# hzdr/PARIS

Hardware: AMD Instinct MI355X
Metric: GVoxel-updates/s (voxels x projections / s), FDK hot path weight+filter+backproject (higher is better)
Workload: dtype f32

## Files before the change

include/paris_hip.h:

```cpp
#ifndef PARIS_HIP_H_
#define PARIS_HIP_H_

#include <stddef.h>
#include <stdint.h>

#ifdef __cplusplus
extern "C" {
#endif

#define PARIS_HIP_SUCCESS 0
#define PARIS_HIP_ERROR_INVALID_ARGUMENT 10001
#define PARIS_HIP_ERROR_NO_DEVICE 10002
#define PARIS_HIP_ERROR_UNSUPPORTED 10003

#define PARIS_HIP_CTX_DEFAULT 0u
#define PARIS_HIP_CTX_SYNCHRONOUS 1u
#define PARIS_HIP_CTX_LEGACY_STREAM 2u
#define PARIS_HIP_CTX_WARM 4u

typedef struct paris_detector_geometry {
    uint32_t n_row;
    uint32_t n_col;
    float l_px_row;
    float l_px_col;
// ... 215 lines not shown
int paris_hip_stage_backproject(paris_hip_ctx* ctx, const float* d_p, size_t p_pitch, uint32_t p_dim_x,
                                uint32_t p_dim_y, uint32_t p_idx, float p_phi, float* d_v, uint32_t v_dim_x,
                                uint32_t v_dim_y, uint32_t v_dim_z, uint32_t v_offset,
                                const paris_detector_geometry* det_geo, const paris_volume_geometry* vol_geo,
                                int enable_angles, int enable_roi, const paris_region_of_interest* roi);

int paris_hip_forward_project(paris_hip_ctx* ctx, const float* d_v, uint32_t v_dim_x, uint32_t v_dim_y, uint32_t v_dim_z,
                              uint32_t v_offset, const paris_detector_geometry* det_geo, const paris_volume_geometry* vol_geo,
                              float* d_p, size_t p_pitch, size_t p_stride_bytes, uint32_t n_views, uint32_t p_dim_x,
                              uint32_t p_dim_y, const float* sin_phi, const float* cos_phi, float delta_s, float delta_t,
                              int accumulate);
int paris_hip_stage_forward_project(paris_hip_ctx* ctx, const float* d_v, uint32_t v_dim_x, uint32_t v_dim_y, uint32_t v_dim_z,
                                    uint32_t v_offset, const paris_detector_geometry* det_geo, const paris_volume_geometry* vol_geo,
                                    float* d_p, size_t p_pitch, uint32_t p_dim_x, uint32_t p_dim_y, uint32_t p_idx, float p_phi,
                                    int enable_angles, int accumulate);

const char* paris_hip_strerror(int status);
const char* paris_hip_version(void);
int paris_hip_has_experiments(void);
int paris_hip_last_backproject_ms(paris_hip_ctx* ctx, float* ms);
int paris_hip_backproject_timing_arm(paris_hip_ctx* ctx, uint32_t capacity);
int paris_hip_backproject_timing_collect(paris_hip_ctx* ctx, float* ms, uint32_t max_n, uint32_t* n_out);
int paris_hip_set_backproject_variant(paris_hip_ctx* ctx, int variant);
int paris_hip_set_backproject_tuning(paris_hip_ctx* ctx, int vx, int unroll, int tz, int lds_bytes);
int paris_hip_set_backproject_slice_shape(paris_hip_ctx* ctx, int waves, int row_groups);
int paris_hip_set_backproject_order(paris_hip_ctx* ctx, int order, int nontemporal);
int paris_hip_set_backproject_fast_division(paris_hip_ctx* ctx, int enable);
int paris_hip_set_backproject_vector_staging(paris_hip_ctx* ctx, int enable);
int paris_hip_fast_division_is_exact(paris_hip_ctx* ctx, float divisor, int* exact);
int paris_hip_lean_division_is_exact(paris_hip_ctx* ctx, float d_sd, float d_so, int* exact);
int paris_hip_lean_weighting_is_exact(paris_hip_ctx* ctx, float d_sd, float q_lo, float q_hi, int* exact);
int paris_hip_set_lean_validation(paris_hip_ctx* ctx, int enable);

#ifdef __cplusplus
}
#endif
#endif
```

paris_amd/_lib.py:

```python
import ctypes as C
import os

_HERE = os.path.dirname(os.path.abspath(__file__))
EXPERIMENTS_LIB_PATH = os.path.join(_HERE, "lib", "libparis_hip_experiments.so")
LIB_PATH = os.environ.get("PARIS_HIP_LIBRARY") or os.path.join(_HERE, "lib", "libparis_hip.so")

SUCCESS = 0
ERROR_INVALID_ARGUMENT = 10001
ERROR_NO_DEVICE = 10002
ERROR_UNSUPPORTED = 10003
CTX_DEFAULT = 0
CTX_SYNCHRONOUS = 1
CTX_LEGACY_STREAM = 2
CTX_WARM = 4
PIXEL_U8 = 1
PIXEL_U16 = 2
PIXEL_U32 = 3
PIXEL_F32 = 4


class DetectorGeometry(C.Structure):
    _fields_ = [("n_row", C.c_uint32), ("n_col", C.c_uint32),
                ("l_px_row", C.c_float), ("l_px_col", C.c_float),
                ("delta_s", C.c_float), ("delta_t", C.c_float),
# ... 127 lines not shown
                                          _P(RegionOfInterest), _P(_u32), _P(_u32)]),
    "paris_hip_stage_angle": (C.c_int, [_P(DetectorGeometry), _u32, C.c_int, _f, _P(_f), _P(_f)]),
    "paris_hip_short_scan_check": (C.c_int, [_P(DetectorGeometry), _P(ShortScan), _P(_f)]),
    "paris_hip_short_scan_weight_rows": (C.c_int, [_vp, _vp, _sz, _sz, _u32, _u32, _u32, _u32, _u32, _P(DetectorGeometry), _P(ShortScan),
                                                   _P(_f)]),
    "paris_hip_stage_short_scan_weight": (C.c_int, [_vp, _vp, _sz, _u32, _u32, _P(DetectorGeometry), _P(ShortScan), _u32, C.c_int,
                                                    _f]),
    "paris_hip_offset_detector_check": (C.c_int, [_P(DetectorGeometry), _P(_f)]),
    "paris_hip_offset_detector_weight_rows": (C.c_int, [_vp, _vp, _sz, _sz, _u32, _u32, _u32, _u32, _u32, _P(DetectorGeometry)]),
    "paris_hip_stage_offset_detector_weight": (C.c_int, [_vp, _vp, _sz, _u32, _u32, _P(DetectorGeometry)]),
    "paris_hip_stage_backproject": (C.c_int, [_vp, _vp, _sz, _u32, _u32, _u32, _f, _vp, _u32, _u32, _u32, _u32,
                                              _P(DetectorGeometry), _P(VolumeGeometry), C.c_int, C.c_int,
                                              _P(RegionOfInterest)]),
    "paris_hip_forward_project": (C.c_int, [_vp, _vp, _u32, _u32, _u32, _u32, _P(DetectorGeometry), _P(VolumeGeometry), _vp, _sz, _sz,
                                            _u32, _u32, _u32, _P(_f), _P(_f), _f, _f, C.c_int]),
    "paris_hip_stage_forward_project": (C.c_int, [_vp, _vp, _u32, _u32, _u32, _u32, _P(DetectorGeometry), _P(VolumeGeometry), _vp, _sz,
                                                  _u32, _u32, _u32, _f, C.c_int, C.c_int]),
    "paris_hip_strerror": (C.c_char_p, [C.c_int]),
    "paris_hip_version": (C.c_char_p, []),
    "paris_hip_last_backproject_ms": (C.c_int, [_vp, _P(_f)]),
    "paris_hip_backproject_timing_arm": (C.c_int, [_vp, _u32]),
    "paris_hip_backproject_timing_collect": (C.c_int, [_vp, _P(_f), _u32, _P(_u32)]),
    "paris_hip_set_backproject_variant": (C.c_int, [_vp, C.c_int]),
    "paris_hip_set_backproject_tuning": (C.c_int, [_vp, C.c_int, C.c_int, C.c_int, C.c_int]),
    "paris_hip_set_backproject_order": (C.c_int, [_vp, C.c_int, C.c_int]),
    "paris_hip_set_backproject_slice_shape": (C.c_int, [_vp, C.c_int, C.c_int]),
    "paris_hip_set_backproject_fast_division": (C.c_int, [_vp, C.c_int]),
    "paris_hip_set_backproject_vector_staging": (C.c_int, [_vp, C.c_int]),
    "paris_hip_fast_division_is_exact": (C.c_int, [_vp, _f, _P(C.c_int)]),
}

_lib = None


def load():
    global _lib
    if _lib is None:
        if not os.path.exists(LIB_PATH):
            raise ImportError(
                "paris_amd: %s not found -- build it with `python -c 'import __graft_entry__ as g; g.build()'` "
                "or `make -C paris_amd/csrc`; there is no CPU fallback" % LIB_PATH)
        if os.environ.get("PARIS_AMD_NO_TORCH") != "1":
            try:
                import torch
            except ImportError:
                pass
        lib = C.CDLL(LIB_PATH)
# ... 24 lines not shown
```

paris_amd/backend.py:

```python
import ctypes as C

import numpy as np

from . import _lib
from ._lib import (DefectStats, DetectorGeometry, ParisHipError, RegionOfInterest, ShortScan, SubvolumeGeometry, SubvolumeInfo,
                   VolumeGeometry, check)

__all__ = ["DetectorGeometry", "VolumeGeometry", "SubvolumeGeometry", "RegionOfInterest", "SubvolumeInfo",
           "ParisHipError", "ShortScan", "Projection", "Volume", "FilterBuffer", "Backend", "get_devices", "set_device",
           "calculate_volume_geometry", "apply_roi", "filter_size", "load", "make_volume", "weight", "filter",
           "backproject", "forward_project", "short_scan_check", "offset_detector_check", "DefectPlan", "defect_plan"]


class Projection:

    def __init__(self, buf, dim_x, dim_y, idx=0, phi=0.0, pitch=None, on_device=False, owner=None):
        self.buf = buf
        self.dim_x = dim_x
        self.dim_y = dim_y
        self.idx = idx
        self.phi = phi
        self.pitch = pitch if pitch is not None else dim_x * 4
        self.on_device = on_device
        self._owner = owner
# ... 398 lines not shown
        check(self._L.paris_hip_forward_project(self._ctx, v.ptr, v.dim_x, v.dim_y, v.dim_z, v_offset, C.byref(det_geo), C.byref(vol_geo),
                                                p.ptr, p.pitch, frame_stride, len(sins), p.dim_x, p.dim_y, sins.ctypes.data_as(fp),
                                                coss.ctypes.data_as(fp), delta_s, delta_t, int(bool(accumulate))),
              "paris_hip_forward_project")

    def last_backproject_ms(self):
        ms = C.c_float()
        check(self._L.paris_hip_last_backproject_ms(self._ctx, C.byref(ms)), "paris_hip_last_backproject_ms")
        return ms.value

    def backproject_timing_arm(self, capacity):
        check(self._L.paris_hip_backproject_timing_arm(self._ctx, capacity), "paris_hip_backproject_timing_arm")

    def backproject_timing_collect(self, max_n=65536):
        ms = (C.c_float * max_n)()
        n = C.c_uint32()
        check(self._L.paris_hip_backproject_timing_collect(self._ctx, ms, max_n, C.byref(n)),
              "paris_hip_backproject_timing_collect")
        return list(ms[:n.value])

    def set_backproject_variant(self, variant):
        check(self._L.paris_hip_set_backproject_variant(self._ctx, variant), "paris_hip_set_backproject_variant")

    def set_backproject_order(self, order=-1, nontemporal=-1):
        check(self._L.paris_hip_set_backproject_order(self._ctx, order, nontemporal), "paris_hip_set_backproject_order")

    def fast_division_is_exact(self, divisor):
        ok = C.c_int()
        check(self._L.paris_hip_fast_division_is_exact(self._ctx, divisor, C.byref(ok)), "paris_hip_fast_division_is_exact")
        return bool(ok.value)

    def set_backproject_vector_staging(self, enable=True):
        check(self._L.paris_hip_set_backproject_vector_staging(self._ctx, int(bool(enable))),
              "paris_hip_set_backproject_vector_staging")

    def set_backproject_fast_division(self, enable=True):
        check(self._L.paris_hip_set_backproject_fast_division(self._ctx, int(bool(enable))),
              "paris_hip_set_backproject_fast_division")

    def set_backproject_slice_shape(self, waves=0, row_groups=0):
        check(self._L.paris_hip_set_backproject_slice_shape(self._ctx, waves, row_groups),
              "paris_hip_set_backproject_slice_shape")

    def set_filter_window(self, window):
        check(self._L.paris_hip_set_filter_window(self._ctx, window), "paris_hip_set_filter_window")

# ... 168 lines not shown
```

paris_amd/csrc/backproject.hip:

```cpp
#include "bp_device.h"

#include <mutex>
#include <utility>

namespace
{
    __global__ void __launch_bounds__(256) fastdiv_validate_kernel(float c, float r, unsigned long long* mismatches)
    {
        const uint32_t t = blockIdx.x * 256u + threadIdx.x;
        unsigned int bad = 0;
        for(uint32_t i = 0; i < 256u; ++i)
        {
            const uint32_t bits = (i << 24) | t;
            const float x = __uint_as_float(bits);
            const float want = x / c - (1.f / 2.f);
            const float got = div_by_constant(x, c, r) - (1.f / 2.f);
            const bool same = __float_as_uint(want) == __float_as_uint(got);
            const bool both_nan = (want != want) && (got != got);
            const bool want_far = !(fabsf(want) <= 16777216.f);
            const bool got_far = !(fabsf(got) <= 16777216.f);
            if(!(same || both_nan || (want_far && got_far)))
                ++bad;
        }
        if(bad)
            atomicAdd(mismatches, static_cast<unsigned long long>(bad));
    }

#ifndef PARIS_TILE_MIN_WAVES
#define PARIS_TILE_MIN_WAVES 1
#endif
    template <int VX, int UNROLL, bool NT, bool FD, bool PRE = false>
    __global__ void __launch_bounds__(256, PARIS_TILE_MIN_WAVES) bp_tile_kernel(const BpParams g)
    {
        extern __shared__ __attribute__((aligned(16))) float lds[];

        constexpr uint32_t XL = 64u / VX;
        constexpr uint32_t RW = VX;
        constexpr uint32_t TY = 4u * RW;

        const uint32_t tid = threadIdx.x;
        const uint32_t lane = tid & 63u;
        const uint32_t wave = tid >> 6;

        uint32_t bx, by, bz;
        if(!tile_of_block(g, blockIdx.x, bx, by, bz))
            return;
        const uint32_t k0 = bx * 64u;
        const uint32_t l0 = by * TY;
        const uint32_t m0 = bz * g.tz;
        const uint32_t k1 = min(k0 + 63u, g.v_dim_x - 1u);
        const uint32_t l1 = min(l0 + TY - 1u, g.v_dim_y - 1u);
        const uint32_t m1 = min(m0 + g.tz - 1u, g.v_dim_z - 1u);

        const uint32_t xq = lane % XL;
        const uint32_t yy = lane / XL;
        const uint32_t k = k0 + xq * VX;
        const uint32_t l = l0 + wave * RW + yy;
        const bool active = k < g.v_dim_x && l < g.v_dim_y;

        float4 pre_f = make_float4(0.f, 0.f, 0.f, 0.f), pre_h = pre_f, pre_u = pre_f;
        if(PRE && VX == 4)
        {
            const size_t plane = static_cast<size_t>(g.v_dim_x) * g.v_dim_y;
            const size_t at = static_cast<size_t>(min(l, l1)) * g.v_dim_x + min(k, g.v_dim_x - 4u);
            pre_f = *reinterpret_cast<const float4*>(g.colstate + at);
            pre_h = *reinterpret_cast<const float4*>(g.colstate + plane + at);
            pre_u = *reinterpret_cast<const float4*>(g.colstate + 2u * plane + at);
        }
// ... 64 lines not shown
                    for(int i = 0; i < UNROLL; ++i)
                        acc[i] = load_voxels<VX, NT>(vp + (mm + i) * slice);
#pragma unroll
                    for(int i = 0; i < UNROLL; ++i)
                        update(acc[i], mm + i);
#pragma unroll
                    for(int i = 0; i < UNROLL; ++i)
                        store_voxels<VX, NT>(vp + (mm + i) * slice, acc[i], g.store_sc1 != 0u);
                }
                for(; mm < mcount; ++mm)
                {
                    vec_t acc = load_voxels<VX, NT>(vp + mm * slice);
                    update(acc, mm);
                    store_voxels<VX, NT>(vp + mm * slice, acc, g.store_sc1 != 0u);
                }
            }
        };
        if(all_fast)
            walk(std::true_type{});
        else
            walk(std::false_type{});
    }

#ifdef PARIS_HIP_EXPERIMENTS
#include "experiments/bp_kernels.inc"
#endif
    __global__ void __launch_bounds__(256) bp_gather_kernel(const BpParams g)
    {
        const uint32_t k = blockIdx.x * 256u + threadIdx.x;
        const uint32_t l = blockIdx.y;
        const uint32_t m = blockIdx.z;
        if(k >= g.v_dim_x)
            return;
        const ColConst c = column_constants<false>(g, g.k_off + k, g.l_off + l);
        const float z_m = g.z_base + static_cast<float>(g.m_off + m) * g.l_vx_z;
        const float x = c.h;
        const float y = v_coordinate<false>(g, z_m, c.factor);
        const float x1 = floorf(x), x2 = x1 + 1.f, y1 = floorf(y), y2 = y1 + 1.f;
        float interp = 0.f;
        if(x1 >= 0.f && x2 < g.p_dim_x_f && y1 >= 0.f && y2 < g.p_dim_y_f)
        {
            const size_t at = static_cast<size_t>(static_cast<uint32_t>(y1)) * g.p_pitch + static_cast<uint32_t>(x1);
            const float q11 = read_pixel(g, at), q21 = read_pixel(g, at + 1);
            const float q12 = read_pixel(g, at + g.p_pitch), q22 = read_pixel(g, at + g.p_pitch + 1);
            const float interp_y1 = (x2 - x) / (x2 - x1) * q11 + (x - x1) / (x2 - x1) * q21;
            const float interp_y2 = (x2 - x) / (x2 - x1) * q12 + (x - x1) / (x2 - x1) * q22;
            interp = (y2 - y) / (y2 - y1) * interp_y1 + (y - y1) / (y2 - y1) * interp_y2;
        }
        float* out = g.vol + (static_cast<size_t>(m) * g.v_dim_y + l) * g.v_dim_x + k;
        *out += 0.5f * interp * c.u * c.u;
    }

    inline float centered_base(uint32_t dim, float size)
    {
        const float size2 = size / 2.f;
        return -(static_cast<float>(dim) * size2) + size2;
    }

    inline float detector_min(uint32_t dim, float size, float offset)
    {
        const float size2 = size / 2.f;
        return -(static_cast<float>(dim) * size2) - offset;
    }

    constexpr uint32_t TZ_DEFAULT = 16;
    constexpr uint32_t LDS_BYTES_DEFAULT = 24u * 1024u;
    constexpr uint32_t LDS_BYTES_MAX = 64u * 1024u;

    template <int VX, int UNROLL, bool NT, bool FD>
    void launch_tile(BpParams& g, hipStream_t stream)
    {
        constexpr uint32_t TY = 4u * VX;
        g.ntx = (g.v_dim_x + 63u) / 64u;
        g.nty = (g.v_dim_y + TY - 1u) / TY;
        g.ntz = (g.v_dim_z + g.tz - 1u) / g.tz;
        settle_order(g);
        g.zchunk = chunk_tiles(g.order, g.tz, g.ntz, 64u);
        const uint32_t blocks = static_cast<uint32_t>(grid_blocks(g));
        hipLaunchKernelGGL((bp_tile_kernel<VX, UNROLL, NT, FD>), dim3(blocks), dim3(256), g.lds_floats * sizeof(float), stream, g);
    }

    template <int VX, bool NT, bool FD>
    void launch_tile_unroll(BpParams& g, int unroll, hipStream_t stream)
    {
        switch(unroll)
        {
            case 1: launch_tile<VX, 1, NT, FD>(g, stream); break;
#ifdef PARIS_HIP_EXPERIMENTS
            case 3: launch_tile<VX, 3, NT, FD>(g, stream); break;
            case 4: launch_tile<VX, 4, NT, FD>(g, stream); break;
#endif
            default: launch_tile<VX, 2, NT, FD>(g, stream); break;
        }
    }

    template <int VX>
    void launch_tile_flags(BpParams& g, int unroll, bool nt, bool fd, hipStream_t stream)
    {
        if(nt && fd)
            launch_tile_unroll<VX, true, true>(g, unroll, stream);
        else if(nt)
            launch_tile_unroll<VX, true, false>(g, unroll, stream);
        else if(fd)
            launch_tile_unroll<VX, false, true>(g, unroll, stream);
        else
            launch_tile_unroll<VX, false, false>(g, unroll, stream);
    }

#ifdef PARIS_HIP_EXPERIMENTS
#include "experiments/bp_launchers.inc"
#endif
    std::mutex fastdiv_mutex;
    std::map<std::pair<int, uint32_t>, bool> fastdiv_cache;

    void fastdiv_enqueue(hipStream_t s, unsigned long long* counter, const void* arg)
    {
        const float c = *static_cast<const float*>(arg);
        hipLaunchKernelGGL(fastdiv_validate_kernel, dim3(1u << 16), dim3(256), 0, s, c, 1.f / c, counter);
    }

    int fastdiv_is_exact(paris_hip_ctx* ctx, float c, bool* ok)
    {
        *ok = false;
        if(!(c > 0.f) || !(c < INFINITY))
            return PARIS_HIP_SUCCESS;
        uint32_t key;
        static_assert(sizeof(key) == sizeof(c), "fp32");
        std::memcpy(&key, &c, sizeof(key));
        auto it = ctx->fastdiv_exact.find(key);
// ... 161 lines not shown
    if(v_dim_x % 2u == 0 && addr % 8u == 0)
        return 2;
    return 1;
}

static int backproject_impl(paris_hip_ctx* ctx, const void* d_p, bool f16, size_t p_pitch, uint32_t p_dim_x,
                            uint32_t p_dim_y, float* d_v, uint32_t v_dim_x, uint32_t v_dim_y, uint32_t v_dim_z,
                            uint32_t v_offset, const paris_detector_geometry* det_geo,
                            const paris_volume_geometry* vol_geo, int enable_roi, const paris_region_of_interest* roi,
                            float sin_phi, float cos_phi, float delta_s, float delta_t)
{
    BpParams g;
    bool fd = false, skip = false;
    if(int rc = fill_params(ctx, d_p, f16, p_pitch, p_dim_x, p_dim_y, d_v, v_dim_x, v_dim_y, v_dim_z, v_offset, det_geo, vol_geo,
                            enable_roi, roi, sin_phi, cos_phi, delta_s, delta_t, g, fd, skip))
        return rc;
    if(skip)
        return paris_hip_finish(ctx);

    const bool timed = !ctx->bp_start.empty();
    const size_t ev = timed ? static_cast<size_t>(ctx->bp_launches % ctx->bp_start.size()) : 0u;
    if(timed)
        PARIS_HIP_TRY(hipEventRecord(ctx->bp_start[ev], ctx->stream));
    if(ctx->bp_variant == 4 && !f16)
    {
        FusedParams fp{};
        fp.g = g;
        fp.n_proj = 1;
        fp.proj_tab[0] = d_p;
        fp.sin_phi[0] = sin_phi;
        fp.cos_phi[0] = cos_phi;
        const int width = lane_width(d_v, v_dim_x);
        const int vx = ctx->bp_vx == 4 && width == 4 ? 4 : (ctx->bp_vx == 1 || width < 2 ? 1 : 2);
        paris_hip_bp_launch_fused(&fp, vx, ctx->bp_tz == 8u ? 8 : (ctx->bp_tz == 32u ? 32 : 16), volume_stream_policy(ctx, v_dim_x, v_dim_y, v_dim_z) != 0, fd, ctx->stream);
    }
    else
    if(ctx->bp_variant == 1)
    {
        const dim3 grid((v_dim_x + 255u) / 256u, v_dim_y, v_dim_z);
        if(v_dim_y > 65535u || v_dim_z > 65535u)
            return PARIS_HIP_ERROR_UNSUPPORTED;
        hipLaunchKernelGGL(bp_gather_kernel, grid, dim3(256), 0, ctx->stream, g);
    }
    else
    {
        int vx = lane_width(d_v, v_dim_x);
        if(ctx->bp_vx && ctx->bp_vx < vx)
            vx = ctx->bp_vx;
        if(ctx->bp_vx == 0 && vx == 4 && ctx->bp_variant != 3 && ctx->bp_variant != 5)
        {
            const uint64_t tiles = static_cast<uint64_t>((v_dim_x + 63u) / 64u) * ((v_dim_y + 15u) / 16u) * ((v_dim_z + g.tz - 1u) / g.tz);
            if(tiles < 2048u)
                vx = 2;
        }
        const bool deep_big = g.tz == 16u && ctx->bp_tz == 0u && static_cast<uint64_t>(v_dim_x) * v_dim_y > (1ull << 20);
        if(deep_big && ctx->bp_unroll == 0 && ctx->bp_lds_bytes == 0u && vx == 4)
            g.lds_floats = 40u * 1024u / sizeof(float);
        const int unroll = ctx->bp_unroll ? ctx->bp_unroll : ((g.tz == 8u && ctx->bp_tz == 0u) || (deep_big && ctx->bp_lds_bytes == 0u && vx == 4) ? 1 : 2);
        const bool nt = volume_stream_policy(ctx, v_dim_x, v_dim_y, v_dim_z) != 0;
#ifdef PARIS_HIP_EXPERIMENTS
        const bool want_slice = ctx->bp_variant == 3;
        if(want_slice && vx == 4)
        {
            const int nw = ctx->bp_slice_nw ? ctx->bp_slice_nw : 16;
            const int rpl = ctx->bp_slice_rpl ? ctx->bp_slice_rpl : 4;
            const uint32_t box_bytes = ctx->bp_lds_bytes ? ctx->bp_lds_bytes : LDS_BYTES_DEFAULT;
            if(int rc = launch_slice_shape(g, nw, rpl, box_bytes, nt, fd, ctx->stream))
                return rc;
        }
        else if(vx == 4 && ctx->bp_variant == 5 && v_dim_y <= 65535u)
        {
            const size_t need = 3u * static_cast<size_t>(v_dim_x) * v_dim_y;
            if(ctx->colstate_floats < need)
            {
                if(ctx->colstate != nullptr)
                {
                    PARIS_HIP_TRY(hipStreamSynchronize(ctx->stream));
                    PARIS_HIP_TRY(hipFree(ctx->colstate));
                    ctx->colstate = nullptr;
                }
                PARIS_HIP_TRY(hipMalloc(reinterpret_cast<void**>(&ctx->colstate), need * sizeof(float)));
                ctx->colstate_floats = need;
            }
            g.colstate = ctx->colstate;
            if(unroll == 1)
                fd ? launch_tile_pre<1, true>(g, ctx->stream) : launch_tile_pre<1, false>(g, ctx->stream);
            else
                fd ? launch_tile_pre<2, true>(g, ctx->stream) : launch_tile_pre<2, false>(g, ctx->stream);
        }
        else
#endif
        if(vx == 4)
            launch_tile_flags<4>(g, unroll, nt, fd, ctx->stream);
        else if(vx == 2)
            launch_tile_flags<2>(g, unroll, nt, fd, ctx->stream);
        else
            launch_tile_flags<1>(g, unroll, nt, fd, ctx->stream);
    }
    if(timed)
        PARIS_HIP_TRY(hipEventRecord(ctx->bp_stop[ev], ctx->stream));
    ++ctx->bp_launches;
    if(int rc = paris_hip_note_projection_use(ctx, d_p, p_pitch * p_dim_y))
        return rc;
    return paris_hip_finish(ctx);
}

static int batch_impl(paris_hip_ctx* ctx, const void* d_p, bool f16, size_t p_pitch, size_t p_stride_bytes, uint32_t n_proj, uint32_t p_dim_x,
                      uint32_t p_dim_y, float* d_v, uint32_t v_dim_x, uint32_t v_dim_y, uint32_t v_dim_z, uint32_t v_offset,
                      const paris_detector_geometry* det_geo, const paris_volume_geometry* vol_geo, int enable_roi,
                      const paris_region_of_interest* roi, const float* sin_phi, const float* cos_phi, float delta_s, float delta_t,
                      const void* const* ptrs = nullptr);

int paris_hip_launch_deferred(paris_hip_ctx* ctx)
{
    if(ctx != nullptr && ctx->pending_weight.active)
        if(int rc = paris_hip_flush_pending_weight(ctx))
            return rc;
    if(ctx == nullptr || ctx->defer_count == 0)
        return PARIS_HIP_SUCCESS;
    const uint32_t n = ctx->defer_count;
// ... 604 lines not shown
                return rc;
    }
    return paris_hip_finish(ctx);
}

extern "C" int paris_hip_last_backproject_ms(paris_hip_ctx* ctx, float* ms)
{
    if(int rc = paris_hip_flush_deferred(ctx))
        return rc;
    if(ctx == nullptr || ms == nullptr || ctx->bp_launches == 0 || ctx->bp_start.empty())
        return PARIS_HIP_ERROR_INVALID_ARGUMENT;
    if(int rc = paris_hip_bind(ctx))
        return rc;
    const size_t ev = static_cast<size_t>((ctx->bp_launches - 1) % ctx->bp_start.size());
    PARIS_HIP_TRY(hipEventSynchronize(ctx->bp_stop[ev]));
    PARIS_HIP_TRY(hipEventElapsedTime(ms, ctx->bp_start[ev], ctx->bp_stop[ev]));
    return PARIS_HIP_SUCCESS;
}

extern "C" int paris_hip_set_backproject_variant(paris_hip_ctx* ctx, int variant)
{
    if(int rc = paris_hip_flush_deferred(ctx))
        return rc;
    if(ctx == nullptr || variant < 0 || variant > 5)
        return PARIS_HIP_ERROR_INVALID_ARGUMENT;
#ifndef PARIS_HIP_EXPERIMENTS
    if(variant == 3 || variant == 5)
        return PARIS_HIP_ERROR_UNSUPPORTED;
#endif
    ctx->bp_variant = variant;
    return PARIS_HIP_SUCCESS;
}

extern "C" int paris_hip_set_backproject_order(paris_hip_ctx* ctx, int order, int nontemporal)
{
    if(int rc = paris_hip_flush_deferred(ctx))
        return rc;
    if(ctx == nullptr || !(order == -1 || order == 0 || order == 1 || order == 5 || order == 8 || order == 9 || order == 12 || (order >= 14 && order <= 18)) || nontemporal < -1 || nontemporal > 2)
        return PARIS_HIP_ERROR_INVALID_ARGUMENT;
#ifndef PARIS_HIP_EXPERIMENTS
    if(order == 0 || order == 1 || order == 8 || order == 9 || order == 12)
        return PARIS_HIP_ERROR_UNSUPPORTED;
#endif
    ctx->bp_order = order;
    ctx->bp_nt = nontemporal;
    return PARIS_HIP_SUCCESS;
}

extern "C" int paris_hip_fast_division_is_exact(paris_hip_ctx* ctx, float divisor, int* exact)
{
    if(int rc = paris_hip_bind(ctx))
        return rc;
    if(exact == nullptr)
// ... 93 lines not shown
```

paris_amd/csrc/bp_device.h:

```cpp
#ifndef PARIS_HIP_BP_DEVICE_H_
#define PARIS_HIP_BP_DEVICE_H_

#include "paris_hip_internal.h"
#include "ieee_lean.h"

#include <algorithm>
#include <cmath>
#include <cstdlib>
#include <cstring>
#include <type_traits>

#ifndef PARIS_BP_SINGLE_INSTRUCTION_FLOOR
#define PARIS_BP_SINGLE_INSTRUCTION_FLOOR 0
#endif

namespace
{
    struct BpParams
    {
        const void* proj;
        uint32_t proj_f16;
        float* vol;
        uint32_t p_pitch;
        uint32_t p_dim_x, p_dim_y;
        uint32_t v_dim_x, v_dim_y, v_dim_z;
        uint32_t k_off, l_off, m_off;
        float x_base, y_base, z_base;
        float l_vx_x, l_vx_y, l_vx_z;
        float sin_phi, cos_phi;
        float d_so, d_sd;
        float min_h, min_v;
        float l_px_x, l_px_y;
        float rcp_l_px_y;
        float rcp_l_px_x;
        float p_dim_x_f, p_dim_y_f;
        uint32_t lds_floats;
        uint32_t tz;
        uint32_t ntx, nty, ntz;
        uint32_t order;
        uint32_t zchunk;
        uint32_t lean_div;
        const float* colstate;
        uint32_t store_sc1;
        uint32_t stage_vec4;
        uint32_t skip_invalid;
        uint32_t yfast;
    };

    struct ColConst
    {
        float factor, h, u;
    };

    __device__ __forceinline__ float div_by_constant(float x, float c, float r)
    {
        const float q = x * r;
        const float e = __builtin_fmaf(-q, c, x);
        return __builtin_fmaf(e, r, q);
    }

    template <bool FD>
    __device__ __forceinline__ ColConst column_constants(const BpParams& g, uint32_t K, uint32_t L)
    {
        const float x_k = g.x_base + static_cast<float>(K) * g.l_vx_x;
        const float y_l = g.y_base + static_cast<float>(L) * g.l_vx_y;
        const float s = x_k * g.cos_phi + y_l * g.sin_phi;
        const float t = -x_k * g.sin_phi + y_l * g.cos_phi;
        const float den = s + g.d_so;
        ColConst c;
        float so_over_den;
// ... 172 lines not shown
            if(g.yfast == 1u)
            {
                by = r % g.nty;
                r /= g.nty;
                bx = r % g.ntx;
                bz = (r / g.ntx) * 8u + xcd;
            }
            else
            {
                bx = r % g.ntx;
                r /= g.ntx;
                by = r % g.nty;
                bz = (r / g.nty) * 8u + xcd;
            }
            return bz < g.ntz;
        }
        if(g.order >= 14u && g.order <= 17u)
        {
            const uint32_t band = dealt_band(g.nty, g.order);
            const uint32_t grp = 1u << (g.order - 14u);
            const uint32_t zchunk = g.zchunk;
            const uint32_t xcd = b % 8u;
            uint32_t r = b / 8u;
            uint32_t zl, yb;
            if(g.yfast == 2u)
            {
                bx = r % g.ntx;
                r /= g.ntx;
                const uint32_t yl = r % grp;
                r /= grp;
                zl = r % zchunk;
                r /= zchunk;
                const uint32_t ngrp = band / grp;
                yb = (r % ngrp) * grp + yl;
                bz = (r / ngrp) * zchunk + zl;
            }
            else if(g.yfast == 1u)
            {
                const uint32_t yl = r % grp;
                r /= grp;
                bx = r % g.ntx;
                r /= g.ntx;
                const uint32_t ngrp = band / grp;
                yb = (r % ngrp) * grp + yl;
                r /= ngrp;
                zl = r % zchunk;
                bz = (r / zchunk) * zchunk + zl;
            }
            else
            {
                bx = r % g.ntx;
                r /= g.ntx;
                zl = r % zchunk;
                r /= zchunk;
                yb = r % band;
                bz = (r / band) * zchunk + zl;
            }
            by = (yb / grp) * (8u * grp) + xcd * grp + yb % grp;
            return bz < g.ntz && by < g.nty;
        }
#ifdef PARIS_HIP_EXPERIMENTS
        if(g.order == 12u)
        {
            const uint32_t band = (g.nty + 7u) / 8u;
            const uint32_t zchunk = g.zchunk;
            const uint32_t xcd = b % 8u;
            uint32_t r = b / 8u;
            bx = r % g.ntx;
            r /= g.ntx;
            const uint32_t zl = r % zchunk;
            r /= zchunk;
            const uint32_t yb = r % band;
            bz = (r / band) * zchunk + zl;
            by = xcd * band + yb;
            return bz < g.ntz && by < g.nty;
        }
        if(g.order == 9u)
        {
            const uint32_t band = (g.nty + 7u) / 8u;
            const uint32_t xcd = b % 8u;
            uint32_t r = b / 8u;
// ... 480 lines not shown
```

paris_amd/csrc/capi.hip:

```cpp
#include "paris_hip_internal.h"
#include <cstdlib>

#include <algorithm>
#include <cstring>
#include <new>

namespace
{
    int physical_device_count(int* count)
    {
        int n = 0;
        const hipError_t err = hipGetDeviceCount(&n);
        if(err == hipErrorNoDevice)
        {
            *count = 0;
            return PARIS_HIP_SUCCESS;
        }
        PARIS_HIP_TRY(err);
        *count = n;
        return PARIS_HIP_SUCCESS;
    }

    int virtual_devices()
    {
// ... 322 lines not shown
    }
    for(auto& p : ctx->pending_checks)
        (void)hipEventDestroy(p.done);
    if(ctx->aux_counter != nullptr)
        (void)hipFree(ctx->aux_counter);
    if(ctx->aux_result != nullptr)
        (void)hipHostFree(ctx->aux_result);
    for(auto& kv : ctx->plans)
    {
        (void)hipFree(kv.second.d_twiddle);
        if(kv.second.d_tab_first != nullptr)
            (void)hipFree(kv.second.d_tab_first);
        for(float2* t : kv.second.d_tab_mid)
            if(t != nullptr)
                (void)hipFree(t);
    }
    for(auto& kv : ctx->filters)
        if(kv.second.d_kp != nullptr)
            (void)hipFree(kv.second.d_kp);
    if(ctx->d_sincos != nullptr)
        (void)hipFree(ctx->d_sincos);
    if(ctx->colstate != nullptr)
        (void)hipFree(ctx->colstate);
    for(auto& kv : ctx->proj_pool)
    {
        if(kv.second.released != nullptr)
            (void)hipEventDestroy(kv.second.released);
        (void)hipFree(kv.second.ptr);
    }
    for(auto& z : ctx->defer_zombies)
        (void)hipFree(z.first);
    for(hipEvent_t e : ctx->group_events)
        if(e != nullptr)
            (void)hipEventDestroy(e);
    for(auto& kv : ctx->host_pool)
    {
        if(kv.second.released != nullptr)
            (void)hipEventDestroy(kv.second.released);
        (void)hipHostFree(kv.second.ptr);
    }
    for(auto& kv : ctx->upload_targets)
        (void)hipEventDestroy(kv.second.last_use);
    for(hipEvent_t e : ctx->spare_events)
        (void)hipEventDestroy(e);
    if(ctx->defer_ring != nullptr)
        (void)hipFree(ctx->defer_ring);
// ... 975 lines not shown
```

paris_amd/csrc/paris_hip_internal.h:

```cpp
#ifndef PARIS_HIP_INTERNAL_H_
#define PARIS_HIP_INTERNAL_H_

#include <hip/hip_runtime.h>

#include <cstddef>
#include <array>
#include <cstdint>
#include <map>
#include <vector>

#include "paris_hip.h"

#pragma clang fp contract(off)

#define PARIS_HIP_TRY(expr)                                   \
    do                                                        \
    {                                                         \
        hipError_t paris_hip_err__ = (expr);                  \
        if(paris_hip_err__ != hipSuccess)                     \
            return static_cast<int>(paris_hip_err__);         \
    } while(0)

struct paris_hip_fft_plan
{
// ... 147 lines not shown
    float* defer_ring = nullptr;
    size_t defer_pitch = 0;
    uint32_t defer_dim_x = 0, defer_dim_y = 0, defer_slots = 0;
    bool defer_f16 = false;
    float* key_v = nullptr;
    bool key_valid = false;
    uint32_t key_dims[4] = {0, 0, 0, 0};
    paris_detector_geometry key_det{};
    paris_volume_geometry key_vol{};
    int key_enable_roi = 0;
    paris_region_of_interest key_roi{};
    float key_delta_s = 0.f, key_delta_t = 0.f;
    std::vector<float> defer_sin, defer_cos;
    int bp_overlap = 0;
    hipStream_t bp_stream = nullptr;
    hipEvent_t bp_ring_ready = nullptr;
    hipEvent_t bp_half_done[2] = {nullptr, nullptr};
    bool bp_half_busy[2] = {false, false};
    bool bp_inflight = false;
    uint32_t bp_last_half = 0;
    uint32_t defer_half = 0;
    float* colstate = nullptr;
    size_t colstate_floats = 0;
    float* d_sincos = nullptr;
    uint32_t d_sincos_cap = 0;
};

inline int paris_hip_finish(paris_hip_ctx* ctx)
{
    PARIS_HIP_TRY(hipGetLastError());
    if(ctx->flags & PARIS_HIP_CTX_SYNCHRONOUS)
        PARIS_HIP_TRY(hipStreamSynchronize(ctx->stream));
    return PARIS_HIP_SUCCESS;
}

inline void paris_hip_mark_touched(paris_hip_ctx* ctx, const void* d_p)
{
    if(ctx->proj_allocs.empty())
        return;
    auto a = ctx->proj_allocs.upper_bound(const_cast<void*>(d_p));
    if(a == ctx->proj_allocs.begin())
        return;
    --a;
    if(static_cast<const char*>(d_p) < static_cast<const char*>(a->first) + a->second.bytes)
        a->second.touched = true;
}
// ... 90 lines not shown
```

Baseline: 786.7.

## Rotate XCD tile ownership per z-chunk and add optional live-tile list backprojection

Adds a rotation of the XCD-to-y-band mapping by z-chunk, which is on by default for large planes, so each XCD's share of live tiles evens out when parts of the volume fall outside the detector. It also adds an opt-in path made of three kernels: one maps live tiles per z-slab, one compacts them per XCD, and one deals them out in a balanced way so the tile kernel walks only live tiles. The list path stays off by default (BP_LIST_DEFAULT false). Rotation changes which XCD's L2 sees which rows, which may cost cache locality.

```diff
diff --git a/include/paris_hip.h b/include/paris_hip.h
--- a/include/paris_hip.h
+++ b/include/paris_hip.h
@@ -261,6 +261,7 @@
 int paris_hip_backproject_timing_arm(paris_hip_ctx* ctx, uint32_t capacity);
 int paris_hip_backproject_timing_collect(paris_hip_ctx* ctx, float* ms, uint32_t max_n, uint32_t* n_out);
 int paris_hip_set_backproject_variant(paris_hip_ctx* ctx, int variant);
+int paris_hip_backproject_live_tiles(paris_hip_ctx* ctx, uint32_t* tiles, uint32_t* listed, uint32_t* xcd_least, uint32_t* xcd_greatest);
 int paris_hip_set_backproject_tuning(paris_hip_ctx* ctx, int vx, int unroll, int tz, int lds_bytes);
 int paris_hip_set_backproject_slice_shape(paris_hip_ctx* ctx, int waves, int row_groups);
 int paris_hip_set_backproject_order(paris_hip_ctx* ctx, int order, int nontemporal);
diff --git a/paris_amd/_lib.py b/paris_amd/_lib.py
--- a/paris_amd/_lib.py
+++ b/paris_amd/_lib.py
@@ -173,7 +173,8 @@
     "paris_hip_backproject_timing_arm": (C.c_int, [_vp, _u32]),
     "paris_hip_backproject_timing_collect": (C.c_int, [_vp, _P(_f), _u32, _P(_u32)]),
     "paris_hip_set_backproject_variant": (C.c_int, [_vp, C.c_int]),
-    "paris_hip_set_backproject_tuning": (C.c_int, [_vp, C.c_int, C.c_int, C.c_int, C.c_int]),
+    "paris_hip_backproject_live_tiles": (C.c_int, [_vp, _P(_u32), _P(_u32), _P(_u32), _P(_u32)]),
+    "paris_hip_set_backproject_tuning":(C.c_int, [_vp, C.c_int, C.c_int, C.c_int, C.c_int]),
     "paris_hip_set_backproject_order": (C.c_int, [_vp, C.c_int, C.c_int]),
     "paris_hip_set_backproject_slice_shape": (C.c_int, [_vp, C.c_int, C.c_int]),
     "paris_hip_set_backproject_fast_division": (C.c_int, [_vp, C.c_int]),
diff --git a/paris_amd/backend.py b/paris_amd/backend.py
--- a/paris_amd/backend.py
+++ b/paris_amd/backend.py
@@ -444,6 +444,11 @@
     def set_backproject_variant(self, variant):
         check(self._L.paris_hip_set_backproject_variant(self._ctx, variant), "paris_hip_set_backproject_variant")
 
+    def backproject_live_tiles(self):
+        v = [C.c_uint32() for _ in range(4)]
+        check(self._L.paris_hip_backproject_live_tiles(self._ctx, *[C.byref(x) for x in v]), "paris_hip_backproject_live_tiles")
+        return tuple(x.value for x in v)
+
     def set_backproject_order(self, order=-1, nontemporal=-1):
         check(self._L.paris_hip_set_backproject_order(self._ctx, order, nontemporal), "paris_hip_set_backproject_order")
 
diff --git a/paris_amd/csrc/backproject.hip b/paris_amd/csrc/backproject.hip
--- a/paris_amd/csrc/backproject.hip
+++ b/paris_amd/csrc/backproject.hip
@@ -29,7 +29,7 @@
 #ifndef PARIS_TILE_MIN_WAVES
 #define PARIS_TILE_MIN_WAVES 1
 #endif
-    template <int VX, int UNROLL, bool NT, bool FD, bool PRE = false>
+    template <int VX, int UNROLL, bool NT, bool FD, bool PRE = false, bool LIST = false>
     __global__ void __launch_bounds__(256, PARIS_TILE_MIN_WAVES) bp_tile_kernel(const BpParams g)
     {
         extern __shared__ __attribute__((aligned(16))) float lds[];
@@ -43,7 +43,13 @@
         const uint32_t wave = tid >> 6;
 
         uint32_t bx, by, bz;
-        if(!tile_of_block(g, blockIdx.x, bx, by, bz))
+        if constexpr(LIST)
+        {
+            if(blockIdx.x >= g.live_info[0])
+                return;
+            unpack_tile(g.live_list[blockIdx.x], bx, by, bz);
+        }
+        else if(!tile_of_block(g, blockIdx.x, bx, by, bz))
             return;
         const uint32_t k0 = bx * 64u;
         const uint32_t l0 = by * TY;
@@ -154,6 +160,172 @@
             walk(std::false_type{});
     }
 
+
+    template <bool FD>
+    __global__ void __launch_bounds__(256) bp_live_map_kernel(const BpParams g, uint8_t* __restrict__ map)
+    {
+        __shared__ float s_fmin[4], s_fmax[4];
+        __shared__ uint32_t s_flags[4];
+        const uint32_t tid = threadIdx.x;
+        const uint32_t lane = tid & 63u;
+        const uint32_t wave = tid >> 6;
+        const uint32_t bx = blockIdx.x % g.ntx, by = blockIdx.x / g.ntx;
+        const uint32_t k0 = bx * 64u, l0 = by * 16u;
+        const uint32_t k1 = min(k0 + 63u, g.v_dim_x - 1u);
+        const uint32_t l1 = min(l0 + 15u, g.v_dim_y - 1u);
+        const uint32_t k = k0 + (lane % 16u) * 4u;
+        const uint32_t l = l0 + wave * 4u + lane / 16u;
+        float fmin = INFINITY, fmax = -INFINITY;
+        uint32_t flags = 0u;
+#pragma unroll
+        for(uint32_t j = 0; j < 4u; ++j)
+        {
+            const ColConst c = column_constants<FD>(g, g.k_off + min(k + j, k1), g.l_off + min(l, l1));
+            const float x1 = floorf(c.h);
+            const float x2 = x1 + 1.f;
+            const bool x_valid = (x1 >= 0.f) && (x2 < g.p_dim_x_f);
+            const bool finite = (c.u - c.u) == 0.f && (c.factor - c.factor) == 0.f;
+            flags |= (x_valid ? 1u : 0u) | (finite ? 0u : 2u);
+            if(x_valid)
+            {
+                fmin = fminf(fmin, c.factor);
+                fmax = fmaxf(fmax, c.factor);
+            }
+        }
+#pragma unroll
+        for(int m = 32; m >= 1; m >>= 1)
+        {
+            fmin = fminf(fmin, __shfl_xor(fmin, m));
+            fmax = fmaxf(fmax, __shfl_xor(fmax, m));
+            flags |= __shfl_xor(flags, m);
+        }
+        if(lane == 0u)
+        {
+            s_fmin[wave] = fmin;
+            s_fmax[wave] = fmax;
+            s_flags[wave] = flags;
+        }
+        __syncthreads();
+        fmin = fminf(fminf(s_fmin[0], s_fmin[1]), fminf(s_fmin[2], s_fmin[3]));
+        fmax = fmaxf(fmaxf(s_fmax[0], s_fmax[1]), fmaxf(s_fmax[2], s_fmax[3]));
+        flags = s_flags[0] | s_flags[1] | s_flags[2] | s_flags[3];
+        for(uint32_t bz = tid; bz < g.ntz; bz += 256u)
+        {
+            const uint32_t m0 = bz * g.tz;
+            const uint32_t m1 = min(m0 + g.tz - 1u, g.v_dim_z - 1u);
+            const float z_first = g.z_base + static_cast<float>(g.m_off + m0) * g.l_vx_z;
+            const float z_last = g.z_base + static_cast<float>(g.m_off + m1) * g.l_vx_z;
+            bool live = (flags & 2u) != 0u;
+            if(!live && (flags & 1u) != 0u)
+            {
+                const float v0 = v_coordinate<FD>(g, z_first, fmin), v1 = v_coordinate<FD>(g, z_last, fmin);
+                const float v2 = v_coordinate<FD>(g, z_first, fmax), v3 = v_coordinate<FD>(g, z_last, fmax);
+                const float top = g.p_dim_y_f - 1.f;
+                const bool below = v0 < 0.f && v1 < 0.f && v2 < 0.f && v3 < 0.f;
+                const bool above = v0 >= top && v1 >= top && v2 >= top && v3 >= top;
+                live = !(below || above);
+            }
+            map[(static_cast<size_t>(bz) * g.nty + by) * g.ntx + bx] = live ? 1u : 0u;
+        }
+    }
+
+    __global__ void __launch_bounds__(1024) bp_live_compact_kernel(const BpParams g, const uint8_t* __restrict__ map, uint32_t per,
+                                                                    uint32_t* __restrict__ own, uint32_t* __restrict__ counts)
+    {
+        __shared__ uint32_t s_wave[16];
+        const uint32_t xcd = blockIdx.x;
+        const uint32_t tid = threadIdx.x;
+        const uint32_t lane = tid & 63u;
+        const uint32_t wave = tid >> 6;
+        const uint32_t run = (per + 1023u) / 1024u;
+        const uint32_t r0 = min(tid * run, per);
+        const uint32_t r1 = min(r0 + run, per);
+        auto live_at = [&](uint32_t r, uint32_t& e) {
+            uint32_t bx, by, bz;
+            if(!tile_of_block(g, 8u * r + xcd, bx, by, bz))
+                return false;
+            e = pack_tile(bx, by, bz);
+            return map[(static_cast<size_t>(bz) * g.nty + by) * g.ntx + bx] != 0u;
+        };
+        uint32_t n = 0u;
+        for(uint32_t r = r0; r < r1; ++r)
+        {
+            uint32_t e;
+            n += live_at(r, e) ? 1u : 0u;
+        }
+        uint32_t incl = n;
+#pragma unroll
+        for(uint32_t d = 1u; d < 64u; d <<= 1)
+        {
+            const uint32_t t = __shfl_up(incl, d);
+            if(lane >= d)
+                incl += t;
+        }
+        if(lane == 63u)
+            s_wave[wave] = incl;
+        __syncthreads();
+        uint32_t base = 0u, total = 0u;
+        for(uint32_t w = 0; w < 16u; ++w)
+        {
+            base += w < wave ? s_wave[w] : 0u;
+            total += s_wave[w];
+        }
+        uint32_t at = base + incl - n;
+        for(uint32_t r = r0; r < r1; ++r)
+        {
+            uint32_t e;
+            if(live_at(r, e))
+            {
+                own[8u * at + xcd] = e;
+                ++at;
+            }
+        }
+        if(tid == 0u)
+            counts[xcd] = total;
+    }
+
+    __global__ void __launch_bounds__(256) bp_live_deal_kernel(const uint32_t* __restrict__ own, const uint32_t* __restrict__ counts,
+                                                                uint32_t all_tiles, uint32_t* __restrict__ list, uint32_t* __restrict__ info)
+    {
+        uint32_t c[8], least = 0xffffffffu, sum = 0u;
+#pragma unroll
+        for(int k = 0; k < 8; ++k)
+        {
+            c[k] = counts[k];
+            least = min(least, c[k]);
+            sum += c[k];
+        }
+        const uint32_t e = blockIdx.x * 256u + threadIdx.x;
+        if(e == 0u)
+        {
+            info[0] = sum;
+            info[1] = all_tiles;
+            info[2] = sum / 8u;
+            info[3] = (sum + 7u) / 8u;
+        }
+        if(e >= sum)
+            return;
+        uint32_t src = e;
+        if(e >= 8u * least)
+        {
+            uint32_t j = e - 8u * least;
+            bool found = false;
+#pragma unroll
+            for(int k = 0; k < 8; ++k)
+            {
+                const uint32_t extra = c[k] - least;
+                if(!found && j < extra)
+                {
+                    src = 8u * (least + j) + static_cast<uint32_t>(k);
+                    found = true;
+                }
+                if(!found)
+                    j -= extra;
+            }
+        }
+        list[e] = own[src];
+    }
+
 #ifdef PARIS_HIP_EXPERIMENTS
 #include "experiments/bp_kernels.inc"
 #endif
@@ -199,8 +371,55 @@
     constexpr uint32_t LDS_BYTES_DEFAULT = 24u * 1024u;
     constexpr uint32_t LDS_BYTES_MAX = 64u * 1024u;
 
+    constexpr int BP_VARIANT_LIST = 6;
+    [[maybe_unused]] constexpr int BP_VARIANT_PLAIN = 7;
+    constexpr int BP_VARIANT_ROTATE_ONLY = 8;
+    constexpr int BP_VARIANT_LIST_ONLY = 9;
+    constexpr bool BP_ROTATE_DEFAULT = true;
+    constexpr bool BP_LIST_DEFAULT = false;
+
+    struct LiveBuffers
+    {
+        uint8_t* map;
+        uint32_t* own;
+        uint32_t* list;
+        uint32_t* counts;
+        uint32_t* info;
+    };
+
+    bool live_buffers(paris_hip_ctx* ctx, uint64_t tiles, uint64_t blocks, hipStream_t stream, LiveBuffers& lb)
+    {
+        const size_t map_bytes = (static_cast<size_t>(tiles) + 255u) & ~static_cast<size_t>(255u);
+        const size_t list_bytes = (static_cast<size_t>(blocks) * sizeof(uint32_t) + 255u) & ~static_cast<size_t>(255u);
+        const size_t need = map_bytes + 2u * list_bytes + 256u;
+        if(ctx->live_bytes < need)
+        {
+            hipStreamCaptureStatus cap = hipStreamCaptureStatusNone;
+            const bool known = hipStreamIsCapturing(stream, &cap) == hipSuccess;
+            (void)hipGetLastError();
+            if(!known || cap != hipStreamCaptureStatusNone)
+                return false;
+            void* p = nullptr;
+            if(hipMalloc(&p, need) != hipSuccess)
+            {
+                (void)hipGetLastError();
+                return false;
+            }
+            if(ctx->live_buf != nullptr)
+                ctx->live_retired.push_back(ctx->live_buf);
+            ctx->live_buf = static_cast<uint8_t*>(p);
+            ctx->live_bytes = need;
+        }
+        lb.map = ctx->live_buf;
+        lb.own = reinterpret_cast<uint32_t*>(ctx->live_buf + map_bytes);
+        lb.list = reinterpret_cast<uint32_t*>(ctx->live_buf + map_bytes + list_bytes);
+        lb.counts = reinterpret_cast<uint32_t*>(ctx->live_buf + map_bytes + 2u * list_bytes);
+        lb.info = lb.counts + 8;
+        return true;
+    }
+
     template <int VX, int UNROLL, bool NT, bool FD>
-    void launch_tile(BpParams& g, hipStream_t stream)
+    void launch_tile(BpParams& g, hipStream_t stream, paris_hip_ctx* ctx, bool want_list)
     {
         constexpr uint32_t TY = 4u * VX;
         g.ntx = (g.v_dim_x + 63u) / 64u;
@@ -209,34 +428,54 @@
         settle_order(g);
         g.zchunk = chunk_tiles(g.order, g.tz, g.ntz, 64u);
         const uint32_t blocks = static_cast<uint32_t>(grid_blocks(g));
+        const uint64_t tiles = static_cast<uint64_t>(g.ntx) * g.nty * g.ntz;
+        ctx->live_last_info = nullptr;
+        ctx->live_last_tiles = static_cast<uint32_t>(tiles);
+        if constexpr(VX == 4)
+        {
+            LiveBuffers lb;
+            if(want_list && g.order >= 14u && g.order <= 17u && g.skip_invalid != 0u && g.ntx <= LIVE_MAX_TX && g.nty <= LIVE_MAX_TY
+               && g.ntz <= LIVE_MAX_TZ && live_buffers(ctx, tiles, blocks, stream, lb))
+            {
+                hipLaunchKernelGGL((bp_live_map_kernel<FD>), dim3(g.ntx * g.nty), dim3(256), 0, stream, g, lb.map);
+                hipLaunchKernelGGL(bp_live_compact_kernel, dim3(8), dim3(1024), 0, stream, g, lb.map, blocks / 8u, lb.own, lb.counts);
+                hipLaunchKernelGGL(bp_live_deal_kernel, dim3((blocks + 255u) / 256u), dim3(256), 0, stream, lb.own, lb.counts,
+                                   static_cast<uint32_t>(tiles), lb.list, lb.info);
+                g.live_list = lb.list;
+                g.live_info = lb.info;
+                ctx->live_last_info = lb.info;
+                hipLaunchKernelGGL((bp_tile_kernel<VX, UNROLL, NT, FD, false, true>), dim3(blocks), dim3(256), g.lds_floats * sizeof(float), stream, g);
+                return;
+            }
+        }
         hipLaunchKernelGGL((bp_tile_kernel<VX, UNROLL, NT, FD>), dim3(blocks), dim3(256), g.lds_floats * sizeof(float), stream, g);
     }
 
     template <int VX, bool NT, bool FD>
-    void launch_tile_unroll(BpParams& g, int unroll, hipStream_t stream)
+    void launch_tile_unroll(BpParams& g, int unroll, hipStream_t stream, paris_hip_ctx* ctx, bool want_list)
     {
         switch(unroll)
         {
-            case 1: launch_tile<VX, 1, NT, FD>(g, stream); break;
+            case 1: launch_tile<VX, 1, NT, FD>(g, stream, ctx, want_list); break;
 #ifdef PARIS_HIP_EXPERIMENTS
-            case 3: launch_tile<VX, 3, NT, FD>(g, stream); break;
-            case 4: launch_tile<VX, 4, NT, FD>(g, stream); break;
+            case 3: launch_tile<VX, 3, NT, FD>(g, stream, ctx, false); break;
+            case 4: launch_tile<VX, 4, NT, FD>(g, stream, ctx, false); break;
 #endif
-            default: launch_tile<VX, 2, NT, FD>(g, stream); break;
+            default: launch_tile<VX, 2, NT, FD>(g, stream, ctx, want_list); break;
         }
     }
 
     template <int VX>
-    void launch_tile_flags(BpParams& g, int unroll, bool nt, bool fd, hipStream_t stream)
+    void launch_tile_flags(BpParams& g, int unroll, bool nt, bool fd, hipStream_t stream, paris_hip_ctx* ctx, bool want_list)
     {
         if(nt && fd)
-            launch_tile_unroll<VX, true, true>(g, unroll, stream);
+            launch_tile_unroll<VX, true, true>(g, unroll, stream, ctx, want_list);
         else if(nt)
-            launch_tile_unroll<VX, true, false>(g, unroll, stream);
+            launch_tile_unroll<VX, true, false>(g, unroll, stream, ctx, want_list);
         else if(fd)
-            launch_tile_unroll<VX, false, true>(g, unroll, stream);
+            launch_tile_unroll<VX, false, true>(g, unroll, stream, ctx, want_list);
         else
-            launch_tile_unroll<VX, false, false>(g, unroll, stream);
+            launch_tile_unroll<VX, false, false>(g, unroll, stream, ctx, want_list);
     }
 
 #ifdef PARIS_HIP_EXPERIMENTS
@@ -444,6 +683,7 @@
     const size_t ev = timed ? static_cast<size_t>(ctx->bp_launches % ctx->bp_start.size()) : 0u;
     if(timed)
         PARIS_HIP_TRY(hipEventRecord(ctx->bp_start[ev], ctx->stream));
+    ctx->live_last_info = nullptr;
     if(ctx->bp_variant == 4 && !f16)
     {
         FusedParams fp{};
@@ -469,12 +709,17 @@
         int vx = lane_width(d_v, v_dim_x);
         if(ctx->bp_vx && ctx->bp_vx < vx)
             vx = ctx->bp_vx;
-        if(ctx->bp_vx == 0 && vx == 4 && ctx->bp_variant != 3 && ctx->bp_variant != 5)
+        const bool list_forced = ctx->bp_variant == BP_VARIANT_LIST || ctx->bp_variant == BP_VARIANT_LIST_ONLY;
+        if(ctx->bp_vx == 0 && vx == 4 && ctx->bp_variant != 3 && ctx->bp_variant != 5 && !list_forced)
         {
             const uint64_t tiles = static_cast<uint64_t>((v_dim_x + 63u) / 64u) * ((v_dim_y + 15u) / 16u) * ((v_dim_z + g.tz - 1u) / g.tz);
             if(tiles < 2048u)
                 vx = 2;
         }
+        const bool big_plane = static_cast<uint64_t>(v_dim_x) * v_dim_y > (1ull << 20);
+        const int variant = ctx->bp_variant;
+        g.rotate = (variant == BP_VARIANT_LIST || variant == BP_VARIANT_ROTATE_ONLY || (variant == 0 && big_plane && BP_ROTATE_DEFAULT)) ? 1u : 0u;
+        const bool want_list = list_forced || (variant == 0 && big_plane && BP_LIST_DEFAULT);
         const bool deep_big = g.tz == 16u && ctx->bp_tz == 0u && static_cast<uint64_t>(v_dim_x) * v_dim_y > (1ull << 20);
         if(deep_big && ctx->bp_unroll == 0 && ctx->bp_lds_bytes == 0u && vx == 4)
             g.lds_floats = 40u * 1024u / sizeof(float);
@@ -513,11 +758,11 @@
         else
 #endif
         if(vx == 4)
-            launch_tile_flags<4>(g, unroll, nt, fd, ctx->stream);
+            launch_tile_flags<4>(g, unroll, nt, fd, ctx->stream, ctx, want_list);
         else if(vx == 2)
-            launch_tile_flags<2>(g, unroll, nt, fd, ctx->stream);
+            launch_tile_flags<2>(g, unroll, nt, fd, ctx->stream, ctx, false);
         else
-            launch_tile_flags<1>(g, unroll, nt, fd, ctx->stream);
+            launch_tile_flags<1>(g, unroll, nt, fd, ctx->stream, ctx, false);
     }
     if(timed)
         PARIS_HIP_TRY(hipEventRecord(ctx->bp_stop[ev], ctx->stream));
@@ -1168,13 +1413,34 @@
 {
     if(int rc = paris_hip_flush_deferred(ctx))
         return rc;
-    if(ctx == nullptr || variant < 0 || variant > 5)
+    if(ctx == nullptr || variant < 0 || variant > BP_VARIANT_LIST_ONLY)
         return PARIS_HIP_ERROR_INVALID_ARGUMENT;
 #ifndef PARIS_HIP_EXPERIMENTS
     if(variant == 3 || variant == 5)
         return PARIS_HIP_ERROR_UNSUPPORTED;
 #endif
     ctx->bp_variant = variant;
+    return PARIS_HIP_SUCCESS;
+}
+
+extern "C" int paris_hip_backproject_live_tiles(paris_hip_ctx* ctx, uint32_t* tiles, uint32_t* listed, uint32_t* xcd_least, uint32_t* xcd_greatest)
+{
+    if(int rc = paris_hip_flush_deferred(ctx))
+        return rc;
+    if(ctx == nullptr || tiles == nullptr || listed == nullptr || xcd_least == nullptr || xcd_greatest == nullptr)
+        return PARIS_HIP_ERROR_INVALID_ARGUMENT;
+    if(int rc = paris_hip_bind(ctx))
+        return rc;
+    uint32_t info[4] = {0u, ctx->live_last_tiles, 0u, 0u};
+    if(ctx->live_last_info != nullptr)
+    {
+        PARIS_HIP_TRY(hipMemcpyAsync(info, ctx->live_last_info, sizeof(info), hipMemcpyDeviceToHost, ctx->stream));
+        PARIS_HIP_TRY(hipStreamSynchronize(ctx->stream));
+    }
+    *listed = info[0];
+    *tiles = info[1];
+    *xcd_least = info[2];
+    *xcd_greatest = info[3];
     return PARIS_HIP_SUCCESS;
 }
 
diff --git a/paris_amd/csrc/bp_device.h b/paris_amd/csrc/bp_device.h
--- a/paris_amd/csrc/bp_device.h
+++ b/paris_amd/csrc/bp_device.h
@@ -45,7 +45,22 @@
         uint32_t stage_vec4;
         uint32_t skip_invalid;
         uint32_t yfast;
+        uint32_t rotate;
+        const uint32_t* live_list;
+        const uint32_t* live_info;
     };
+
+    constexpr uint32_t LIVE_MAX_TX = 1u << 10, LIVE_MAX_TY = 1u << 11, LIVE_MAX_TZ = 1u << 11;
+    __host__ __device__ inline uint32_t pack_tile(uint32_t bx, uint32_t by, uint32_t bz)
+    {
+        return bx | (by << 10) | (bz << 21);
+    }
+    __host__ __device__ inline void unpack_tile(uint32_t e, uint32_t& bx, uint32_t& by, uint32_t& bz)
+    {
+        bx = e & 1023u;
+        by = (e >> 10) & 2047u;
+        bz = e >> 21;
+    }
 
     struct ColConst
     {
@@ -264,7 +279,7 @@
             const uint32_t zchunk = g.zchunk;
             const uint32_t xcd = b % 8u;
             uint32_t r = b / 8u;
-            uint32_t zl, yb;
+            uint32_t zl, yb, chunk = 0u;
             if(g.yfast == 2u)
             {
                 bx = r % g.ntx;
@@ -275,7 +290,8 @@
                 r /= zchunk;
                 const uint32_t ngrp = band / grp;
                 yb = (r % ngrp) * grp + yl;
-                bz = (r / ngrp) * zchunk + zl;
+                chunk = r / ngrp;
+                bz = chunk * zchunk + zl;
             }
             else if(g.yfast == 1u)
             {
@@ -296,9 +312,11 @@
                 zl = r % zchunk;
                 r /= zchunk;
                 yb = r % band;
-                bz = (r / band) * zchunk + zl;
-            }
-            by = (yb / grp) * (8u * grp) + xcd * grp + yb % grp;
+                chunk = r / band;
+                bz = chunk * zchunk + zl;
+            }
+            const uint32_t owner = g.rotate != 0u ? (xcd + chunk) % 8u : xcd;
+            by = (yb / grp) * (8u * grp) + owner * grp + yb % grp;
             return bz < g.ntz && by < g.nty;
         }
 #ifdef PARIS_HIP_EXPERIMENTS
diff --git a/paris_amd/csrc/capi.hip b/paris_amd/csrc/capi.hip
--- a/paris_amd/csrc/capi.hip
+++ b/paris_amd/csrc/capi.hip
@@ -368,6 +368,10 @@
         (void)hipFree(ctx->d_sincos);
     if(ctx->colstate != nullptr)
         (void)hipFree(ctx->colstate);
+    if(ctx->live_buf != nullptr)
+        (void)hipFree(ctx->live_buf);
+    for(void* p : ctx->live_retired)
+        (void)hipFree(p);
     for(auto& kv : ctx->proj_pool)
     {
         if(kv.second.released != nullptr)
diff --git a/paris_amd/csrc/paris_hip_internal.h b/paris_amd/csrc/paris_hip_internal.h
--- a/paris_amd/csrc/paris_hip_internal.h
+++ b/paris_amd/csrc/paris_hip_internal.h
@@ -193,6 +193,11 @@
     uint32_t defer_half = 0;
     float* colstate = nullptr;
     size_t colstate_floats = 0;
+    uint8_t* live_buf = nullptr;
+    size_t live_bytes = 0;
+    std::vector<void*> live_retired;
+    const uint32_t* live_last_info = nullptr;
+    uint32_t live_last_tiles = 0;
     float* d_sincos = nullptr;
     uint32_t d_sincos_cap = 0;
 };
```

Result: no change. 790.7 (median of 6 runs) (+0.5%).
